# facebookresearch/generative-recommenders

Hardware: AMD Instinct MI355X
Metric: user-seqs/sec (fwd+bwd) HSTU attention L=200 d=512 (higher is better)
Workload: dtype bf16

## Files before the change

### generative_recommenders_amd/csrc/hstu_attn_bwd_fold.cuh

```cuda
#pragma once
#include "hstu_attn_bwd.cuh"

#ifndef FOLD_SDP_AHEAD
#define FOLD_SDP_AHEAD 3
#endif
#ifndef FOLD_DQ32_AHEAD
#define FOLD_DQ32_AHEAD 2
#endif

namespace hstu {

#pragma clang diagnostic push
#pragma clang diagnostic ignored "-Winline-asm"
HSTU_DEV void dma16_asm(const char* g, uint32_t lds_base) {
  asm volatile("s_mov_b32 m0, %1\n\ts_nop 0\n\tglobal_load_lds_dwordx4 %0, off" HSTU_DMA_POLICY ::"v"(g), "s"(lds_base) : "memory", "m0");
}
#pragma clang diagnostic pop

HSTU_DEV void dma16_saddr(uint32_t off, const char* base, uint32_t lds_base) { dma16_saddr_asm(off, base, lds_base); }

template <typename T, int D>
HSTU_DEV void fold_tile_dma(char* tile, const char* base, int64_t row_stride_bytes, int row0, int len, int wave, int lane, bool fast) {
  constexpr int UPR = D * Elem<T>::kBytes / 16;
  constexpr int NCH = 32 * UPR / 64;
  const uint32_t lds0 = __builtin_amdgcn_readfirstlane((uint32_t)(uintptr_t)tile);
  for (int c = wave; c < NCH; c += kBwdWaves) {
    const int pidx = c * 64 + lane;
    const int row = pidx / UPR, slot = pidx % UPR;
    const int unit = slot ^ swz<UPR>(row);
    const int grow = min(row0 + row, len - 1);
    if (fast) dma16_saddr(__umul24((uint32_t)grow, (uint32_t)row_stride_bytes) + unit * 16, base, lds0 + c * 1024);
    else dma16_asm(base + (int64_t)grow * row_stride_bytes + unit * 16, lds0 + c * 1024);
  }
}

HSTU_DEV int fold_ds_off(int row, int chunk) { return (row << 6) + ((chunk ^ ((row >> 1) & 7)) << 3); }

struct FoldNoBias {
  static constexpr bool on = false;
};
struct FoldBias {
  static constexpr bool on = true;
  BiasCtx bc;
  float* hpos;
  float* hts;
  char* bcache;
  bool cached;
  TsRun ts_run;
};

template <typename T, int DQK, int DV, typename BX = FoldNoBias, bool PUBLISH = true, bool CTXM = false>
HSTU_DEV void fold_pair_x(const HstuAttnParams& p, const MaskCtx& mc, const char* __restrict__ Kw, const char* __restrict__ Vw,
                        const char* __restrict__ Qs, const char* __restrict__ dOs, char* __restrict__ myds, int i0, int k0, f32x16 (&dk_acc)[DQK / 32],
                        f32x16 (&dv_acc)[DV / 32], int lane, int dmvm, BX& bx HSTU_TRACE_ARG) {
  using C = BwdCfg<T, DQK, DV>;
  using E = Elem<T>;
  using Frag = typename E::Frag;
  const int n32 = lane & 31, hf = lane >> 5;
  const int len = mc.len;
  const int key = k0 + n32;
  const bool key_ok = key < len;
  f32x16 s, dp;
  Frag pb[2], dsb[2];
  int mode;
  const bool plain = mc.simple || (mc.has_targets && mc.win == 0 && mc.ctx == 0 && i0 + 32 <= min(len, mc.max_id));
  if (plain) mode = (k0 < i0 && i0 + 32 <= len) ? 0 : 1;
  else mode = (i0 + 32 <= len && mc.pair_fully_valid(i0, 32, k0, 32)) ? 0 : 2;
  const int key_id = mc.id_of(key);
  const int key_bits = key_ok ? -1 : 0;
  auto mask_init = [&]() {
    int km = -1;
    if (mode == 1) km = ((k0 == i0) ? dmvm : -1) & ((i0 + 32 > len) ? (dmvm >> 16) : -1);
    if (mode == 2) {
      km = 0;
      bool ctx_done = false;
      if constexpr (CTXM) {
        if (mc.ctx > 0) {
#pragma unroll
          for (int r = 0; r < 16; ++r) {
            const int qi = i0 + (r & 3) + 8 * (r >> 2) + 4 * hf;
            km |= (((qi < len) & key_ok & mc.valid_ids(qi, key, mc.id_of(qi), key_id)) ? 1 : 0) << r;
          }
          ctx_done = true;
        }
      }
      if (!ctx_done) {
#pragma unroll
        for (int r = 0; r < 16; ++r) {
          const int qi = i0 + (r & 3) + 8 * (r >> 2) + 4 * hf;
          km |= (mc.keep_bits_noctx(qi, key, key_id) & key_bits & 1) << r;
        }
      }
    }
    const unsigned nk = ~(unsigned)km;
    const unsigned neg = __builtin_bit_cast(unsigned, p.alpha < 0.f ? 1e30f : -1e30f);
#pragma unroll
    for (int r = 0; r < 16; ++r) {
      const int m = ((int)(nk << (31 - r))) >> 31;
      s[r] = __builtin_bit_cast(float, (unsigned)m & neg);
    }
  };
#pragma unroll
  for (int r = 0; r < 16; ++r) dp[r] = 0.f;
  static_assert(DQK == DV, "interleaved S / dP stream");
  {
    constexpr int NM = 2 * C::KGQ, AHEAD = FOLD_SDP_AHEAD;
    Frag fa[AHEAD + 1], fb[AHEAD + 1];
    auto load_item = [&](int m, Frag& a, Frag& bb) {
      const int e0 = hf * (DQK / 2) + (m >> 1) * 8;
      a = lds_row_frag<T, C::UPR_K>((m & 1) ? dOs : Qs, n32, e0);
      bb = lds_row_frag<T, C::UPR_K>((m & 1) ? Vw : Kw, n32, e0);
    };
#pragma unroll
    for (int m = 0; m < AHEAD; ++m) load_item(m, fa[m % (AHEAD + 1)], fb[m % (AHEAD + 1)]);
    __builtin_amdgcn_sched_barrier(0);
#pragma unroll
    for (int m = 0; m < NM; ++m) {
      if (m + AHEAD < NM) load_item(m + AHEAD, fa[(m + AHEAD) % (AHEAD + 1)], fb[(m + AHEAD) % (AHEAD + 1)]);
      if (m & 1) dp = E::mma(fa[m % (AHEAD + 1)], fb[m % (AHEAD + 1)], dp);
      else if (m == 0) {
        if (mode == 0) {
          f32x16 z;
#pragma unroll
          for (int r = 0; r < 16; ++r) z[r] = 0.f;
          s = E::mma(fa[0], fb[0], z);
        } else {
          mask_init();
          s = E::mma(fa[0], fb[0], s);
        }
      } else s = E::mma(fa[m % (AHEAD + 1)], fb[m % (AHEAD + 1)], s);
      __builtin_amdgcn_sched_barrier(0);
    }
  }
  HSTU_MARK(11);
  int t_k32 = 0;
  if constexpr (BX::on) {
    if (bx.bc.small) t_k32 = bx.bc.t32_at(key);
  }
  float ds_keep[BX::on ? 16 : 1];
  int bkt_keep[BX::on ? 16 : 1];
  int pbase_keep[2] = {0, 0};
  auto elem = [&](const int h8) {
    float pv[8], dsv[8];
    float xb[8];
    int bkt[8];
    int pbase = 0;
    if constexpr (BX::on) {
      const BiasCtx& bc = bx.bc;
      const int qt = i0 >> 5, kt = k0 >> 5;
      char* const bslot = bx.bcache + ((((qt * (qt + 1)) >> 1) + kt) * 2 + h8) * 512 + 8 * lane;
      if (bx.cached) {
        const u32x2 w = *LDS_PTR(const u32x2, bslot);
#pragma unroll
        for (int j = 0; j < 8; ++j) bkt[j] = (int)((w[j >> 2] >> (8 * (j & 3))) & 255u);
      } else {
        if (bc.small) {
#pragma unroll
          for (int g = 0; g < 2; ++g) {
            const auto t4 = bc.t32x4_next(i0 + 8 * (2 * h8 + g) + 4 * hf);
#pragma unroll
            for (int j = 0; j < 4; ++j) bkt[4 * g + j] = bc.bucket32(t4[j], t_k32);
          }
        } else {
#pragma unroll
          for (int j = 0; j < 8; ++j) {
            const int r = 8 * h8 + j;
            bkt[j] = bc.bucket(bc.ts_at(i0 + (r & 3) + 8 * (r >> 2) + 4 * hf + 1), bc.ts_at(key));
          }
        }
        u32x2 w = {0u, 0u};
#pragma unroll
        for (int j = 0; j < 8; ++j) w[j >> 2] |= (unsigned)bkt[j] << (8 * (j & 3));
        *LDS_PTR(u32x2, bslot) = w;
      }
      pbase = bc.pos_index(i0 + 16 * h8 + 4 * hf, key);
#pragma unroll
      for (int j = 0; j < 8; ++j) xb[j] = bc.value(pbase - (j & 3) - 8 * (j >> 2), bkt[j]);
    }
    {
      const f32x2 a2 = {p.alpha, p.alpha};
      const f32x2 c2 = {-1.44269504088896340736f * p.alpha, -1.44269504088896340736f * p.alpha};
      const f32x2 nl2 = {-1.44269504088896340736f, -1.44269504088896340736f};
      const f32x2 one2 = {1.f, 1.f};
#pragma unroll
      for (int j = 0; j < 8; j += 2) {
        const int r = 8 * h8 + j;
        const f32x2 sv = {s[r], s[r + 1]}, dpv = {dp[r], dp[r + 1]};
        f32x2 x = sv * a2, t = sv * c2;
        if constexpr (BX::on) {
          const f32x2 bv = {xb[j], xb[j + 1]};
          x = x + bv;
          t = x * nl2;
        }
        const f32x2 e = {__builtin_amdgcn_exp2f(t[0]), __builtin_amdgcn_exp2f(t[1])};
        const f32x2 dn = e + one2;
        const f32x2 sg = {__builtin_amdgcn_rcpf(dn[0]), __builtin_amdgcn_rcpf(dn[1])};
        const f32x2 pr = x * sg;
        const f32x2 dsr = dpv * (pr * (one2 - sg) + sg);
        pv[j] = pr[0]; pv[j + 1] = pr[1];
        dsv[j] = dsr[0]; dsv[j + 1] = dsr[1];
      }
    }
    if constexpr (BX::on) {
      pbase_keep[h8] = pbase;
#pragma unroll
      for (int j = 0; j < 8; ++j) { ds_keep[8 * h8 + j] = dsv[j]; bkt_keep[8 * h8 + j] = bkt[j]; }
    }
    pb[h8] = E::pack8(pv);
    dsb[h8] = E::pack8(dsv);
  };
  elem(0);
  elem(1);
  HSTU_MARK(12);
  {
    constexpr int NM = 2 * 2 * C::DBQ, AHEAD = FOLD_SDP_AHEAD;
    Frag fa[AHEAD + 1];
    auto load_item = [&](int m, Frag& a) {
      const int ks = (m >> 1) & 1, d = m >> 2;
      a = lds_col_frag<T, C::UPR_K>((m & 1) ? Qs : dOs, 16 * ks + 4 * hf, 16 * ks + 8 + 4 * hf, 32 * d, lane);
    };
#pragma unroll
    for (int m = 0; m < AHEAD; ++m) load_item(m, fa[m % (AHEAD + 1)]);
    __builtin_amdgcn_sched_barrier(0);
#pragma unroll
    for (int m = 0; m < NM; ++m) {
      if (m + AHEAD < NM) load_item(m + AHEAD, fa[(m + AHEAD) % (AHEAD + 1)]);
      const int ks = (m >> 1) & 1, d = m >> 2;
      if (m & 1) dk_acc[d] = E::mma(fa[m % (AHEAD + 1)], dsb[ks], dk_acc[d]);
      else dv_acc[d] = E::mma(fa[m % (AHEAD + 1)], pb[ks], dv_acc[d]);
      __builtin_amdgcn_sched_barrier(0);
    }
  }
#pragma unroll
  for (int rq = 0; PUBLISH && rq < 4; ++rq) {
    const u32x4 w = __builtin_bit_cast(u32x4, dsb[rq >> 1].v);
    u32x2 v2 = {w[2 * (rq & 1)], w[2 * (rq & 1) + 1]};
    *LDS_PTR(u32x2, myds + fold_ds_off(n32, hf + 2 * rq)) = v2;
  }
  if constexpr (BX::on) {
#pragma unroll
    for (int h8 = 0; h8 < 2; ++h8) {
      const float* dsv_ = ds_keep + 8 * h8;
      const int* bkt_ = bkt_keep + 8 * h8;
      const int pbase_ = pbase_keep[h8];
      const int p16 = lane & 15;
#pragma unroll
      for (int gg = 0; gg < 2; ++gg) {
        float t = dsv_[4 * gg + 3];
#pragma unroll
        for (int j = 2; j >= 0; --j)
          t = __builtin_bit_cast(float, __builtin_amdgcn_update_dpp(0, __builtin_bit_cast(int, t), 0x101, 0xf, 0xf, true)) + dsv_[4 * gg + j];
        if (t != 0.f) atomicAdd(bx.hpos + pbase_ - 8 * gg, t);
#pragma unroll
        for (int j = 1; j < 4; ++j)
          if (p16 < j && dsv_[4 * gg + j] != 0.f) atomicAdd(bx.hpos + pbase_ - 8 * gg - j, dsv_[4 * gg + j]);
      }
      if (bx.bc.lts) {
#pragma unroll
        for (int j = 0; j < 8; ++j) bx.ts_run.add(bkt_[j], dsv_[j]);
      }
    }
  }
}

template <typename T, int DQK, int DV>
HSTU_DEV void fold_pair(const HstuAttnParams& p, const MaskCtx& mc, const char* __restrict__ Kw, const char* __restrict__ Vw,
                        const char* __restrict__ Qs, const char* __restrict__ dOs, char* __restrict__ myds, int i0, int k0, f32x16 (&dk_acc)[DQK / 32],
                        f32x16 (&dv_acc)[DV / 32], int lane, int dmvm HSTU_TRACE_ARG) {
  FoldNoBias nb;
  fold_pair_x<T, DQK, DV, FoldNoBias>(p, mc, Kw, Vw, Qs, dOs, myds, i0, k0, dk_acc, dv_acc, lane, dmvm, nb HSTU_TRACE_PASS);
}

template <typename T, int D>
HSTU_DEV void fold_park_tile(const f32x16 (&acc)[D / 32], float scale, char* __restrict__ tile, int lane) {
  constexpr int UPR = D * Elem<T>::kBytes / 16;
  const int n32 = lane & 31, hf = lane >> 5;
#pragma unroll
  for (int d = 0; d < D / 32; ++d)
#pragma unroll
    for (int rq = 0; rq < 4; ++rq) {
      u32x2 v = {Elem<T>::pk2(acc[d][4 * rq] * scale, acc[d][4 * rq + 1] * scale),
                 Elem<T>::pk2(acc[d][4 * rq + 2] * scale, acc[d][4 * rq + 3] * scale)};
      *LDS_PTR(u32x2, tile + tile_off<UPR>(n32, 4 * d + rq) + 8 * hf) = v;
    }
}
template <typename T, int D, int NT = kBwdThreads>
HSTU_DEV void fold_copy_out(const char* __restrict__ tile, char* gtile, int64_t row_stride_bytes, int rows_valid, int tid) {
  constexpr int UPR = D * Elem<T>::kBytes / 16;
  for (int u = tid; u < 32 * UPR; u += NT) {
    const int row = u / UPR, unit = u % UPR;
    const u32x4 v = *LDS_PTR(const u32x4, tile + tile_off<UPR>(row, unit));
    if (row < rows_valid) gstore16_nt(gtile + row * row_stride_bytes + unit * 16, v);
  }
}

template <int NB>
HSTU_DEV void fold_dump(const f32x16 (&acc)[NB], char* __restrict__ region, int lane) {
#pragma unroll
  for (int d = 0; d < NB; ++d)
#pragma unroll
    for (int c = 0; c < 4; ++c) {
      f32x4 v4 = {acc[d][4 * c], acc[d][4 * c + 1], acc[d][4 * c + 2], acc[d][4 * c + 3]};
      *LDS_PTR(f32x4, region + ((d * 4 + c) * 64 + lane) * 16) = v4;
    }
}
template <int NB>
HSTU_DEV void fold_add(f32x16 (&acc)[NB], const char* __restrict__ region, int lane) {
#pragma unroll
  for (int d = 0; d < NB; ++d)
#pragma unroll
    for (int c = 0; c < 4; ++c) {
      const f32x4 v4 = *LDS_PTR(const f32x4, region + ((d * 4 + c) * 64 + lane) * 16);
#pragma unroll
      for (int e = 0; e < 4; ++e) acc[d][4 * c + e] += v4[e];
    }
}

template <typename T>
HSTU_DEV typename Elem<T>::Frag tr_frag16(const char* base, int off_lo, int off_hi) {
  s16x4 a = __builtin_amdgcn_ds_read_tr16_b64_v4i16(LDS_PTR(s16x4, base + off_lo));
  s16x4 b = __builtin_amdgcn_ds_read_tr16_b64_v4i16(LDS_PTR(s16x4, base + off_hi));
  typedef short s16x8 __attribute__((ext_vector_type(8)));
  s16x8 ab = {a[0], a[1], a[2], a[3], b[0], b[1], b[2], b[3]};
  typename Elem<T>::Frag f;
  f.v = __builtin_bit_cast(typename Elem<T>::vec8, ab);
  return f;
}

template <typename T, int DQK, int DV, int NA, int NB>
HSTU_DEV void fold_dq_slots(char* dq_head, int64_t dq_rs, const MaskCtx& mc, const char* __restrict__ kv,
                            const char* __restrict__ dsbuf, int a, int bq, bool b_on, int wave,
                            float ds_scale, int lane HSTU_TRACE_ARG) {
  using C = BwdCfg<T, DQK, DV>;
  using F = FoldCfg<T, DQK, DV>;
  using E = Elem<T>;
  using Frag = typename E::Frag;
  const int db = wave & 3, qb = wave >> 2;
  if (db >= DQK / 32) return;
  const int i16 = lane & 15, g = lane >> 4;
  const int row_lo = 8 * g + (i16 >> 2), row_hi = row_lo + 4;
  constexpr bool kContig = C::UPR_K == 16;
  const int colK0 = kContig ? 32 * db + 4 * (i16 & 3) : 32 * db + 8 * (i16 & 3), colK1 = colK0 + (kContig ? 16 : 4);
  const int k0_lo = tile_off<C::UPR_K>(row_lo, colK0 >> 3) + ((colK0 & 7) << 1);
  const int k0_hi = tile_off<C::UPR_K>(row_hi, colK0 >> 3) + ((colK0 & 7) << 1);
  const int k1_lo = tile_off<C::UPR_K>(row_lo, colK1 >> 3) + ((colK1 & 7) << 1);
  const int k1_hi = tile_off<C::UPR_K>(row_hi, colK1 >> 3) + ((colK1 & 7) << 1);
  const int d_lo = fold_ds_off(row_lo, 4 * qb + (i16 & 3)), d_hi = fold_ds_off(row_hi, 4 * qb + (i16 & 3));
  unsigned on_a = (1u << (a + 1)) - 1u, on_b = b_on ? (1u << (bq + 1)) - 1u : 0u;
  if (mc.win != 0) {
    for (int t = 0; t <= a; ++t)
      if (!mc.pair_may_be_active(32 * a, 32, 32 * t, 32)) on_a &= ~(1u << t);
    if (b_on)
      for (int t = 0; t <= bq; ++t)
        if (!mc.pair_may_be_active(32 * bq, 32, 32 * t, 32)) on_b &= ~(1u << t);
  }
  HSTU_MARK(19);
  f32x4 acc[2][2];
#pragma unroll
  for (int sd = 0; sd < 2; ++sd)
#pragma unroll
    for (int h = 0; h < 2; ++h) acc[sd][h] = f32x4{0.f, 0.f, 0.f, 0.f};
  const u32x4 zero4 = {0u, 0u, 0u, 0u};
#pragma unroll
  for (int sd = 0; sd < 2; ++sd) {
#pragma unroll
    for (int t = 0; t < (sd ? NB : NA); ++t) {
      const bool on = ((sd ? on_b : on_a) >> t) & 1u;
      const char* Kt = kv + t * C::PAIR;
      const char* ds = dsbuf + (sd ? (kBwdWaves - 1 - t) : t) * F::DSB;
      const Frag fk0 = tr_frag16<T>(Kt, k0_lo, k0_hi), fk1 = tr_frag16<T>(Kt, k1_lo, k1_hi);
      Frag fd = tr_frag16<T>(ds, d_lo, d_hi);
      fd.v = __builtin_bit_cast(typename E::vec8, on ? __builtin_bit_cast(u32x4, fd.v) : zero4);
      acc[sd][0] = E::mma16(fk0, fd, acc[sd][0]);
      acc[sd][1] = E::mma16(fk1, fd, acc[sd][1]);
    }
  }
  {
    constexpr int NSLOT = NA + NB;
    __builtin_amdgcn_sched_group_barrier(0x100, 6, 0);
#pragma unroll
    for (int sl = 0; sl < NSLOT; ++sl) {
      if (sl + 1 < NSLOT) __builtin_amdgcn_sched_group_barrier(0x100, 6, 0);
      __builtin_amdgcn_sched_group_barrier(0x002, 4, 0);
      __builtin_amdgcn_sched_group_barrier(0x008, 2, 0);
    }
  }
  HSTU_MARK(16);
#pragma unroll
  for (int sd = 0; sd < 2; ++sd) {
    if (sd == 1 && !b_on) break;
    uint32_t x0 = E::pk2(acc[sd][0][0] * ds_scale, acc[sd][0][1] * ds_scale), x1 = E::pk2(acc[sd][0][2] * ds_scale, acc[sd][0][3] * ds_scale);
    uint32_t y0 = E::pk2(acc[sd][1][0] * ds_scale, acc[sd][1][1] * ds_scale), y1 = E::pk2(acc[sd][1][2] * ds_scale, acc[sd][1][3] * ds_scale);
    int f0 = 8 * g;
    if constexpr (kContig) {
      const auto s0 = __builtin_amdgcn_permlane16_swap(x0, y0, false, false);
      const auto s1 = __builtin_amdgcn_permlane16_swap(x1, y1, false, false);
      x0 = s0[0]; y0 = s0[1]; x1 = s1[0]; y1 = s1[1];
      f0 = 8 * (2 * (g & 1) + (g >> 1));
    }
    const int qrow = 32 * (sd ? bq : a) + 16 * qb + i16;
    if (qrow < mc.len) gstore16(dq_head + qrow * dq_rs + (32 * db + f0) * C::EB, u32x4{x0, x1, y0, y1});
  }
}

template <typename T, int DQK, int DV>
HSTU_DEV void fold_dq_phase(char* dq_head, int64_t dq_rs, const MaskCtx& mc, const char* __restrict__ kv,
                            const char* __restrict__ dsbuf, int a, int bq, bool b_on, int wave,
                            float ds_scale, int lane HSTU_TRACE_ARG) {
#define HSTU_FOLD_DQ(NA_, NB_) return fold_dq_slots<T, DQK, DV, NA_, NB_>(dq_head, dq_rs, mc, kv, dsbuf, a, bq, b_on, wave, ds_scale, lane HSTU_TRACE_PASS)
  const int code = 8 * (a + 1) + (b_on ? bq + 1 : 0);
  switch (code) {
    case 8 * 7 + 1: HSTU_FOLD_DQ(7, 1);
    case 8 * 6 + 2: HSTU_FOLD_DQ(6, 2);
    case 8 * 5 + 3: HSTU_FOLD_DQ(5, 3);
    case 8 * 4 + 0: HSTU_FOLD_DQ(4, 0);
    default: HSTU_FOLD_DQ(7, 4);
  }
#undef HSTU_FOLD_DQ
}

template <typename T, int D, int N>
HSTU_DEV f32x16 fold_dq_chain32(const char* __restrict__ kv, const char* __restrict__ ds0, int ds_step, int db, int lane) {
  using C = BwdCfg<T, D, D>;
  using E = Elem<T>;
  using Frag = typename E::Frag;
  const int hf = lane >> 5, i16 = lane & 15, g1 = (lane >> 4) & 1;
  const int ra = 8 * hf, rb = 16 + 8 * hf;
  const int chunk = 4 * g1 + (i16 & 3), rr = i16 >> 2;
  const int o00 = fold_ds_off(ra + rr, chunk), o01 = fold_ds_off(ra + 4 + rr, chunk);
  const int o10 = fold_ds_off(rb + rr, chunk), o11 = fold_ds_off(rb + 4 + rr, chunk);
  f32x16 acc;
#pragma unroll
  for (int r = 0; r < 16; ++r) acc[r] = 0.f;
#pragma unroll
  for (int t = 0; t < N; ++t) {
    const char* Kt = kv + t * C::PAIR;
    const char* ds = ds0 + t * ds_step;
    const Frag a0 = lds_col_frag<T, C::UPR_K>(Kt, ra, ra + 4, 32 * db, lane);
    const Frag a1 = lds_col_frag<T, C::UPR_K>(Kt, rb, rb + 4, 32 * db, lane);
    const Frag b0 = tr_frag16<T>(ds, o00, o01);
    const Frag b1 = tr_frag16<T>(ds, o10, o11);
    acc = E::mma(a0, b0, acc);
    acc = E::mma(a1, b1, acc);
  }
  {
    constexpr int AH = FOLD_DQ32_AHEAD < N ? FOLD_DQ32_AHEAD : N;
    __builtin_amdgcn_sched_group_barrier(0x100, 8 * AH, 0);
#pragma unroll
    for (int t = 0; t < N; ++t) {
      if (t + AH < N) __builtin_amdgcn_sched_group_barrier(0x100, 8, 0);
      __builtin_amdgcn_sched_group_barrier(0x008, 2, 0);
    }
  }
  return acc;
}

template <typename T, int D>
HSTU_DEV void fold_dq_phase32(char* dq_head, int64_t dq_rs, const MaskCtx& mc, const char* __restrict__ kv, const char* __restrict__ dsbuf,
                              int a, int bq, bool b_on, int wave, float ds_scale, int lane HSTU_TRACE_ARG) {
  using C = BwdCfg<T, D, D>;
  using F = FoldCfg<T, D, D>;
  using E = Elem<T>;
  static_assert(D == 128, "four feature blocks x two sides = eight waves");
  const int db = wave & 3, side = wave >> 2;
  if (side == 1 && !b_on) return;
  const int n = side ? bq + 1 : a + 1;
  const int q0 = 32 * (side ? bq : a);
  const char* ds0 = side ? dsbuf + (kBwdWaves - 1) * F::DSB : dsbuf;
  const int ds_step = side ? -F::DSB : F::DSB;
  HSTU_MARK(19);
  f32x16 acc;
  switch (n) {
    case 1: acc = fold_dq_chain32<T, D, 1>(kv, ds0, ds_step, db, lane); break;
    case 2: acc = fold_dq_chain32<T, D, 2>(kv, ds0, ds_step, db, lane); break;
    case 3: acc = fold_dq_chain32<T, D, 3>(kv, ds0, ds_step, db, lane); break;
    case 4: acc = fold_dq_chain32<T, D, 4>(kv, ds0, ds_step, db, lane); break;
    case 5: acc = fold_dq_chain32<T, D, 5>(kv, ds0, ds_step, db, lane); break;
    case 6: acc = fold_dq_chain32<T, D, 6>(kv, ds0, ds_step, db, lane); break;
    default: acc = fold_dq_chain32<T, D, 7>(kv, ds0, ds_step, db, lane); break;
  }
  HSTU_MARK(16);
  const int n32 = lane & 31, hf = lane >> 5;
  uint32_t g[4][2];
#pragma unroll
  for (int j = 0; j < 4; ++j) {
    g[j][0] = E::pk2(acc[4 * j] * ds_scale, acc[4 * j + 1] * ds_scale);
    g[j][1] = E::pk2(acc[4 * j + 2] * ds_scale, acc[4 * j + 3] * ds_scale);
  }
#pragma unroll
  for (int jp = 0; jp < 4; jp += 2)
#pragma unroll
    for (int h = 0; h < 2; ++h) {
      const auto sw = __builtin_amdgcn_permlane32_swap(g[jp][h], g[jp + 1][h], false, false);
      g[jp][h] = sw[0];
      g[jp + 1][h] = sw[1];
    }
  const int qrow = q0 + n32;
  if (qrow < mc.len) {
    char* dst = dq_head + qrow * dq_rs + (32 * db + 8 * hf) * C::EB;
    gstore16(dst, u32x4{g[0][0], g[0][1], g[1][0], g[1][1]});
    gstore16(dst + 16 * C::EB, u32x4{g[2][0], g[2][1], g[3][0], g[3][1]});
  }
}


typedef const __attribute__((address_space(4))) uint32_t* kargw_t;
#define HSTU_KARG(k, field) (((const __attribute__((address_space(4))) HstuAttnBwdParams*)(k))->field)

HSTU_DEV HstuAttnBwdParams reload_bwd_params(kargw_t k) {
  static_assert(sizeof(HstuAttnBwdParams) % 4 == 0, "word copy");
  HstuAttnBwdParams r;
  uint32_t* d = (uint32_t*)&r;
#pragma unroll
  for (int i = 0; i < (int)(sizeof(HstuAttnBwdParams) / 4); ++i) d[i] = k[i];
  return r;
}

struct FoldWork {
  int64_t off0;
  int len;
  int b, hd;
};

HSTU_DEV FoldWork fold_work(const HstuAttnParams& p, int uh, int tmax) {
  FoldWork w;
  w.b = user_of_slot_s(p, uh / p.heads);
  w.hd = uh % p.heads;
  w.off0 = sload_index(p.seq_offsets, w.b, p.offsets_dtype);
  w.len = min((int)(sload_index(p.seq_offsets, w.b + 1, p.offsets_dtype) - w.off0), 32 * tmax);
  return w;
}

template <typename T, int DQK, int DV, typename BX = FoldNoBias>
HSTU_DEV void fold_problem_x(const HstuAttnBwdParams& bp, kargw_t kargs, int tmax, const FoldWork& cur, const FoldWork& nxt, char* smem,
                             int tid, int lane, int wave, int& pre_lo, BX& bx) {
  using C = BwdCfg<T, DQK, DV>;
  using F = FoldCfg<T, DQK, DV>;
  static_assert(C::EB == 2, "the folded backward is built for 16-bit I/O");
  static_assert(DQK / 32 <= 4, "dQ GEMM: 32 feature columns x 16 query rows per wave");
  static_assert(DQK == DV, "hand-over regions assume equal K and V tile sizes");
  const HstuAttnParams& p = bp.fwd;
  const int64_t off0 = cur.off0;
  const int len = cur.len, hd = cur.hd;
  const int pre_in = pre_lo;
  pre_lo = F::kMaxTiles;
  if (len <= 0) return;
  const MaskCtx mc = make_mask_ctx<true>(p, cur.b, len);
  HSTU_TRACE_DECL(bp.workspace, bp.workspace != nullptr && cur.b * p.heads + hd == 4096);
  HSTU_MARK(1);

  const int nt = (len + 31) >> 5;
  const int ns = (nt + 1) >> 1;
  char* const stageA = smem + F::kMaxTiles * C::PAIR;
  char* const stageB = stageA + C::PAIR;
  char* const dsbuf = stageB + C::PAIR;

  const char* qbase = (const char*)p.q + (off0 * p.q_row_stride + (int64_t)hd * p.q_head_stride) * C::EB;
  const char* dobase = (const char*)bp.dout + (off0 * bp.do_row_stride + (int64_t)hd * bp.do_head_stride) * C::EB;
  char* const dq_head = (char*)bp.dq + (off0 * bp.dq_row_stride + (int64_t)hd * bp.dq_head_stride) * C::EB;
  char* const dk_head = (char*)bp.dk + (off0 * bp.dk_row_stride + (int64_t)hd * bp.dk_head_stride) * C::EB;
  char* const dv_head = (char*)bp.dv + (off0 * bp.dv_row_stride + (int64_t)hd * bp.dv_head_stride) * C::EB;
  const int64_t dq_rs = bp.dq_row_stride * C::EB, dk_rs = bp.dk_row_stride * C::EB, dv_rs = bp.dv_row_stride * C::EB;
  const int64_t q_rs = p.q_row_stride * C::EB, k_rs = p.k_row_stride * C::EB, v_rs = p.v_row_stride * C::EB,
                do_rs = bp.do_row_stride * C::EB;

  const int len_max = 32 * tmax;
  const bool dma_fast = q_rs < (1 << 24) && k_rs < (1 << 24) && v_rs < (1 << 24) && do_rs < (1 << 24) &&
                        (int64_t)len_max * q_rs < (1LL << 32) && (int64_t)len_max * k_rs < (1LL << 32) &&
                        (int64_t)len_max * v_rs < (1LL << 32) && (int64_t)len_max * do_rs < (1LL << 32);
  auto stage_dma = [&](int qa, int qb, bool b_on) {
    fold_tile_dma<T, DQK>(stageA, qbase, q_rs, 32 * qa, len, wave, lane, dma_fast);
    fold_tile_dma<T, DV>(stageA + C::KT, dobase, do_rs, 32 * qa, len, wave, lane, dma_fast);
    if (b_on) {
      fold_tile_dma<T, DQK>(stageB, qbase, q_rs, 32 * qb, len, wave, lane, dma_fast);
      fold_tile_dma<T, DV>(stageB + C::KT, dobase, do_rs, 32 * qb, len, wave, lane, dma_fast);
    }
  };

  {
    const char* kbase = (const char*)p.k + (off0 * p.k_row_stride + (int64_t)hd * p.k_head_stride) * C::EB;
    const char* vbase = (const char*)p.v + (off0 * p.v_row_stride + (int64_t)hd * p.v_head_stride) * C::EB;
    for (int t = 0; t < min(nt, pre_in); ++t) {
      char* dst = smem + t * C::PAIR;
      fold_tile_dma<T, DQK>(dst, kbase, k_rs, 32 * t, len, wave, lane, dma_fast);
      fold_tile_dma<T, DV>(dst + C::KT, vbase, v_rs, 32 * t, len, wave, lane, dma_fast);
    }
  }
  stage_dma(nt - 1, 0, 0 < nt - 1);
  for (int i = tid; i < kBwdWaves * F::DSB / 16; i += kBwdThreads) *LDS_PTR(u32x4, dsbuf + 16 * i) = u32x4{0u, 0u, 0u, 0u};
  for (int t = nt; t < F::kMaxTiles; ++t)
    for (int i = tid; i < C::KT / 16; i += kBwdThreads) *LDS_PTR(u32x4, smem + t * C::PAIR + 16 * i) = u32x4{0u, 0u, 0u, 0u};
  HSTU_MARK(2);

  f32x16 dk_acc[C::DBQ], dv_acc[C::DBV];
#pragma unroll
  for (int d = 0; d < C::DBQ; ++d)
#pragma unroll
    for (int r = 0; r < 16; ++r) dk_acc[d][r] = 0.f;
#pragma unroll
  for (int d = 0; d < C::DBV; ++d)
#pragma unroll
    for (int r = 0; r < 16; ++r) dv_acc[d][r] = 0.f;
  const float scale_v = attn_scale_of(p);
  const float ds_scale = scale_v * p.alpha;

  int dmvm = 0;
  {
    const int n32 = lane & 31, hf = lane >> 5;
#pragma unroll
    for (int r = 0; r < 16; ++r) {
      const int row = (r & 3) + 8 * (r >> 2) + 4 * hf;
      dmvm |= (n32 <= row ? 1 : 0) << r;
      dmvm |= (32 * (nt - 1) + row < len ? 1 : 0) << (16 + r);
    }
  }

  for (int k = 0; k < ns; ++k) {
    const int a = nt - 1 - k, bq = k;
    const bool b_on = bq < a;
    asm volatile("s_waitcnt vmcnt(0)" ::: "memory");
    __syncthreads();
    HSTU_MARK(10);
    if (k > 0 && wave == a + 1) {
      int lane3 = lane;
      asm volatile("" : "+v"(lane3));
      fold_park_tile<T, DQK>(dk_acc, ds_scale, smem + wave * C::PAIR, lane3);
#pragma unroll
      for (int d = 0; d < C::DBQ; ++d)
#pragma unroll
        for (int r = 0; r < 16; ++r) dk_acc[d][r] = 0.f;
    }
    int kt = -1, qt = 0;
    const char* st = stageA;
    if (wave <= a) { kt = wave; qt = a; }
    else if (b_on && kBwdWaves - 1 - wave <= bq) { kt = kBwdWaves - 1 - wave; qt = bq; st = stageB; }
    if (kt >= 0 && (mc.win == 0 || mc.pair_may_be_active(32 * qt, 32, 32 * kt, 32))) {
      const char* Kw = smem + kt * C::PAIR;
      int lane1 = lane;
      asm volatile("" : "+v"(lane1));
      fold_pair_x<T, DQK, DV, BX>(p, mc, Kw, Kw + C::KT, st, st + C::KT, dsbuf + wave * F::DSB, 32 * qt, 32 * kt, dk_acc,
                                  dv_acc, lane1, dmvm, bx HSTU_TRACE_PASS);
    }
    HSTU_MARK(13);
    HSTU_MARK(14);
    __syncthreads();
    HSTU_MARK(15);
    if (k + 1 < ns) stage_dma(a - 1, bq + 1, bq + 1 < a - 1);
    if (k > 0) {
      const int kt1 = a + 1;
      fold_copy_out<T, DQK>(smem + kt1 * C::PAIR, dk_head + (int64_t)(32 * kt1) * dk_rs, dk_rs, len - 32 * kt1, tid);
      fold_copy_out<T, DV>(smem + kt1 * C::PAIR + C::KT, dv_head + (int64_t)(32 * kt1) * dv_rs, dv_rs, len - 32 * kt1, tid);
    }
    HSTU_MARK(18);
    int lane2 = lane;
    asm volatile("" : "+v"(lane2));
    bool done32 = false;
    if constexpr (DQK == 128 && DV == 128 && !BX::on) {
      if (mc.win == 0) {
        fold_dq_phase32<T, DQK>(dq_head, dq_rs, mc, smem, dsbuf, a, bq, b_on, wave, ds_scale, lane2 HSTU_TRACE_PASS);
        done32 = true;
      }
    }
    if (!done32) fold_dq_phase<T, DQK, DV>(dq_head, dq_rs, mc, smem, dsbuf, a, bq, b_on, wave, ds_scale, lane2 HSTU_TRACE_PASS);
    HSTU_MARK(17);
    if (kt == wave && wave == a) {
      int lane3 = lane;
      asm volatile("" : "+v"(lane3));
      fold_park_tile<T, DV>(dv_acc, scale_v, smem + wave * C::PAIR + C::KT, lane3);
#pragma unroll
      for (int d = 0; d < C::DBV; ++d)
#pragma unroll
        for (int r = 0; r < 16; ++r) dv_acc[d][r] = 0.f;
    }
    HSTU_MARK(23);
  }
  HSTU_MARK(20);
  const int nb = nt >> 1;
  const int a_last = nt - ns;
  const int bt = kBwdWaves - 1 - wave;
  const bool a_fin = wave < nb, b_fin = bt < nb;
  const int tb = a_fin ? wave : bt;
  char* const reg_a = smem + tb * C::PAIR;
  char* const reg_b = tb == 0 ? stageA : (tb == 1 ? stageB : dsbuf);
  __syncthreads();
  if (nxt.len > 0) {
    kargw_t k2 = kargs;
    asm volatile("" : "+s"(k2));
    const int64_t krs3 = HSTU_KARG(k2, fwd.k_row_stride), vrs3 = HSTU_KARG(k2, fwd.v_row_stride);
    const char* kb3 = (const char*)HSTU_KARG(k2, fwd.k) + (nxt.off0 * krs3 + (int64_t)nxt.hd * HSTU_KARG(k2, fwd.k_head_stride)) * C::EB;
    const char* vb3 = (const char*)HSTU_KARG(k2, fwd.v) + (nxt.off0 * vrs3 + (int64_t)nxt.hd * HSTU_KARG(k2, fwd.v_head_stride)) * C::EB;
    const int nt3 = (nxt.len + 31) >> 5;
    for (int t = a_last + 1; t < nt3; ++t) {
      char* dst = smem + t * C::PAIR;
      fold_tile_dma<T, DQK>(dst, kb3, krs3 * C::EB, 32 * t, nxt.len, wave, lane, dma_fast);
      fold_tile_dma<T, DV>(dst + C::KT, vb3, vrs3 * C::EB, 32 * t, nxt.len, wave, lane, dma_fast);
    }
    pre_lo = a_last + 1;
  }
  int lane4 = lane;
  asm volatile("" : "+v"(lane4));
  if (wave == a_last) fold_park_tile<T, DQK>(dk_acc, ds_scale, smem + wave * C::PAIR, lane4);
  if (a_fin) fold_dump<C::DBV>(dv_acc, reg_a, lane4);
  if (b_fin) fold_dump<C::DBQ>(dk_acc, reg_b, lane4);
  __syncthreads();
  HSTU_MARK(22);
  if (a_fin) {
    fold_add<C::DBQ>(dk_acc, reg_b, lane4);
    fold_park_tile<T, DQK>(dk_acc, ds_scale, reg_b, lane4);
  }
  if (b_fin) {
    fold_add<C::DBV>(dv_acc, reg_a, lane4);
    fold_park_tile<T, DV>(dv_acc, scale_v, reg_a + C::KT, lane4);
  }
  __syncthreads();
  HSTU_MARK(24);
  fold_copy_out<T, DQK>(smem + a_last * C::PAIR, dk_head + (int64_t)(32 * a_last) * dk_rs, dk_rs, len - 32 * a_last, tid);
  fold_copy_out<T, DV>(smem + a_last * C::PAIR + C::KT, dv_head + (int64_t)(32 * a_last) * dv_rs, dv_rs, len - 32 * a_last, tid);
  for (int t = 0; t < nb; ++t) {
    const char* rb = t == 0 ? stageA : (t == 1 ? stageB : dsbuf);
    fold_copy_out<T, DQK>(rb, dk_head + (int64_t)(32 * t) * dk_rs, dk_rs, len - 32 * t, tid);
    fold_copy_out<T, DV>(smem + t * C::PAIR + C::KT, dv_head + (int64_t)(32 * t) * dv_rs, dv_rs, len - 32 * t, tid);
  }
  HSTU_MARK(21);
}

template <typename T, int DQK, int DV>
__global__ __launch_bounds__(kBwdThreads) __attribute__((amdgpu_waves_per_eu(2, 2))) void hstu_attn_bwd_fold_kernel(const HstuAttnBwdParams bp_arg, int tmax) {
  extern __shared__ __attribute__((aligned(16))) char smem[];
  const int tid = threadIdx.x;
  const int lane = tid & 63;
  const int wave = __builtin_amdgcn_readfirstlane(tid >> 6);
  const kargw_t kargs = (kargw_t)__builtin_amdgcn_kernarg_segment_ptr();
  const int total = HSTU_KARG(kargs, fwd.batch) * HSTU_KARG(kargs, fwd.heads);
  int pre_lo = 7;
  FoldNoBias nb;
  FoldWork cur;
  {
    const HstuAttnBwdParams bp0 = reload_bwd_params(kargs);
    cur = fold_work(bp0.fwd, blockIdx.x, tmax);
  }
  for (int uh = blockIdx.x; uh < total; uh += gridDim.x) {
    kargw_t kl = kargs;
    asm volatile("" : "+s"(kl));
    const HstuAttnBwdParams bp = reload_bwd_params(kl);
    FoldWork nxt;
    nxt.len = 0; nxt.off0 = 0; nxt.b = 0; nxt.hd = 0;
    if (uh + (int)gridDim.x < total) nxt = fold_work(bp.fwd, uh + (int)gridDim.x, tmax);
    fold_problem_x<T, DQK, DV, FoldNoBias>(bp, kl, tmax, cur, nxt, smem, tid, lane, wave, pre_lo, nb);
    cur = nxt;
    __syncthreads();
  }
}

template <typename T, int D>
__global__ __launch_bounds__(kBwdThreads) __attribute__((amdgpu_waves_per_eu(2, 2))) void hstu_attn_bwd_fold_bias_kernel(
    const HstuAttnBwdParams bp_arg, int tmax, float* bias_partial, int ts_copies, int hist_bytes, int table_bytes, int* next_user) {
  using F = FoldCfg<T, D, D>;
  extern __shared__ __attribute__((aligned(16))) char smem[];
  const int tid = threadIdx.x;
  const int lane = tid & 63;
  const int wave = __builtin_amdgcn_readfirstlane(tid >> 6);
  const kargw_t kargs = (kargw_t)__builtin_amdgcn_kernarg_segment_ptr();
  const int batch = HSTU_KARG(kargs, fwd.batch), heads = HSTU_KARG(kargs, fwd.heads);
  const int max_seq_len = HSTU_KARG(kargs, fwd.max_seq_len), num_buckets = HSTU_KARG(kargs, fwd.num_buckets);
  FoldBias bx;
  bx.hpos = (float*)(smem + F::smem_bytes());
  bx.hts = bx.hpos + 2 * max_seq_len;
  char* const tables = (char*)bx.hpos + hist_bytes;
  bx.bcache = tables + table_bytes;
  bx.ts_run.init(bx.hts, ts_copies);
  bx.cached = false;
  const int hist_floats = 2 * max_seq_len + (num_buckets + 1) * ts_copies;
  for (int i = tid; i < hist_floats; i += kBwdThreads) bx.hpos[i] = 0.f;
  int pre_lo = 7;
  FoldWork cur;
  {
    const HstuAttnBwdParams bp0 = reload_bwd_params(kargs);
    cur = fold_work(bp0.fwd, (int)blockIdx.x * heads, tmax);
  }
  volatile int* const slot = (volatile int*)(bx.hpos + 2 * max_seq_len - 1);
  int ticket = 0;
  if (tid == 0) ticket = (int)gridDim.x + atomicAdd(next_user, 1);
  for (int u = blockIdx.x; u < batch;) {
    if (tid == 0) {
      *slot = ticket;
      ticket = (int)gridDim.x + atomicAdd(next_user, 1);
    }
    __syncthreads();
    {
      kargw_t kl = kargs;
      asm volatile("" : "+s"(kl));
      const HstuAttnBwdParams bp = reload_bwd_params(kl);
      bx.bc = stage_bias_tables(bp.fwd, cur.b, tables, tid, kBwdThreads, u != (int)blockIdx.x);
    }
    __syncthreads();
    bx.bc.finish(kBwdWaves);
    const int u_next = __builtin_amdgcn_readfirstlane(*slot);
    for (int hd = 0; hd < heads; ++hd) {
      kargw_t kl = kargs;
      asm volatile("" : "+s"(kl));
      const HstuAttnBwdParams bp = reload_bwd_params(kl);
      const int uh = u * heads + hd;
      const int uh_n = hd + 1 < heads ? uh + 1 : (u_next < batch ? u_next * heads : -1);
      FoldWork nxt;
      nxt.len = 0; nxt.off0 = 0; nxt.b = 0; nxt.hd = 0;
      if (hd + 1 < heads) { nxt = cur; nxt.hd = hd + 1; }
      else if (uh_n >= 0) nxt = fold_work(bp.fwd, uh_n, tmax);
      bx.cached = hd > 0;
      fold_problem_x<T, D, D, FoldBias>(bp, kl, tmax, cur, nxt, smem, tid, lane, wave, pre_lo, bx);
      cur = nxt;
      __syncthreads();
    }
    u = u_next;
  }
  bx.ts_run.flush();
  __syncthreads();
  const HstuAttnBwdParams bp = reload_bwd_params(kargs);
  const float scale_v = attn_scale_of(bp.fwd);
  float* row = bias_partial + (int64_t)blockIdx.x * (2 * max_seq_len + num_buckets);
  const int npos = 2 * max_seq_len - 1;
  for (int i = tid; i < 2 * max_seq_len + num_buckets; i += kBwdThreads) {
    float v;
    if (i < npos) {
      v = bx.hpos[i];
    } else {
      v = 0.f;
      const float* cp = bx.hts + (i - npos) * ts_copies;
      for (int c = 0; c < ts_copies; ++c) v += cp[c];
    }
    row[i] = v * scale_v;
  }
}

}
```

Measured before the change: 1.922 million.

## Add software-pipelined pair kernel interleaving S/dP, dV and dK MFMA streams

Adds an alternate fold_pair_x path, selected at compile time, that runs the S/dP MMAs and the following dV/dK MMAs as one unrolled stream with fragment loads issued ahead. The sigmoid/P and dS elementwise stages are placed among the MMAs according to a configurable ordering, and dS publication to LDS is delayed. The aim is to hide LDS load latency and elementwise SFU work behind matrix-core work. It is enabled by default with order 3 for DQK=128 without bias, and it raises register pressure from the larger prefetch and staging arrays.

```diff
diff --git a/generative_recommenders_amd/csrc/hstu_attn_bwd_fold.cuh b/generative_recommenders_amd/csrc/hstu_attn_bwd_fold.cuh
--- a/generative_recommenders_amd/csrc/hstu_attn_bwd_fold.cuh
+++ b/generative_recommenders_amd/csrc/hstu_attn_bwd_fold.cuh
@@ -49,7 +49,39 @@
   TsRun ts_run;
 };
 
-template <typename T, int DQK, int DV, typename BX = FoldNoBias, bool PUBLISH = true, bool CTXM = false>
+#ifndef FOLD_PAIR_ORDER
+#define FOLD_PAIR_ORDER 3
+#endif
+#ifndef FOLD_PAIR_PACKED
+#define FOLD_PAIR_PACKED 0
+#endif
+#ifndef FOLD_PAIR_LEAD
+#define FOLD_PAIR_LEAD 3
+#endif
+template <int ORDER, int KGQ, int DB>
+struct FoldPairOrder {
+  static constexpr int NS = 2 * KGQ, ND = 4 * DB, N = NS + ND;
+  static constexpr int L = FOLD_PAIR_LEAD;
+  static constexpr int SLAST = ORDER == 4 ? 2 * KGQ - 2 - L : (ORDER == 1 ? KGQ - 1 : 2 * KGQ - 2);
+  static constexpr int kind(int pos) {
+    if (pos < NS) {
+      if (ORDER == 1) return pos >= KGQ ? 1 : 0;
+      if (ORDER == 4) return pos < L ? 0 : (pos > SLAST ? 1 : ((pos - L) & 1));
+      return pos & 1;
+    }
+    const int m = pos - NS;
+    return 2 + (ORDER == 1 ? (m >= 2 * DB ? 1 : 0) : (m & 1));
+  }
+  static constexpr int kq(int pos) {
+    if (ORDER == 1) return pos % KGQ;
+    if (ORDER == 4) return pos < L ? pos : (pos > SLAST ? KGQ - 1 - L + (pos - SLAST - 1) : (((pos - L) & 1) ? (pos - L - 1) / 2 : L + (pos - L) / 2));
+    return pos >> 1;
+  }
+  static constexpr int d(int pos) { return ORDER == 1 ? (pos - NS) % DB : ((pos - NS) >> 1) % DB; }
+  static constexpr int ks(int pos) { return ORDER == 1 ? ((pos - NS) / DB) & 1 : (pos - NS) / (2 * DB); }
+};
+
+template <typename T, int DQK, int DV, typename BX = FoldNoBias, bool PUBLISH = true, bool CTXM = false, int ORDER = 0>
 HSTU_DEV void fold_pair_x(const HstuAttnParams& p, const MaskCtx& mc, const char* __restrict__ Kw, const char* __restrict__ Vw,
                         const char* __restrict__ Qs, const char* __restrict__ dOs, char* __restrict__ myds, int i0, int k0, f32x16 (&dk_acc)[DQK / 32],
                         f32x16 (&dv_acc)[DV / 32], int lane, int dmvm, BX& bx HSTU_TRACE_ARG) {
@@ -103,6 +135,139 @@
 #pragma unroll
   for (int r = 0; r < 16; ++r) dp[r] = 0.f;
   static_assert(DQK == DV, "interleaved S / dP stream");
+  if constexpr (ORDER != 0) {
+    static_assert(!BX::on && E::kBytes == 2, "pipelined pair: 16-bit I/O, no bias");
+    using PO = FoldPairOrder<ORDER, C::KGQ, C::DBQ>;
+    constexpr int AHEAD = FOLD_SDP_AHEAD, NS = PO::NS, N = PO::N, NG = 2 * C::DBQ;
+    static_assert(16 % C::KGQ == 0 && 16 % NG == 0 && (16 / C::KGQ) % 2 == 0 && (16 / NG) % 2 == 0, "element pairs per slot");
+    Frag fa[AHEAD + 1], fb[AHEAD + 1];
+    float fac[16];
+    uint32_t pw[8], dsw[8];
+    auto load_item = [&](int pos, Frag& a, Frag& bb) {
+      const int kd = PO::kind(pos);
+      if (kd < 2) {
+        const int e0 = hf * (DQK / 2) + PO::kq(pos) * 8;
+        a = lds_row_frag<T, C::UPR_K>(kd ? dOs : Qs, n32, e0);
+        bb = lds_row_frag<T, C::UPR_K>(kd ? Vw : Kw, n32, e0);
+      } else {
+        const int ks = PO::ks(pos), d = PO::d(pos);
+        a = lds_col_frag<T, C::UPR_K>(kd == 3 ? Qs : dOs, 16 * ks + 4 * hf, 16 * ks + 8 + 4 * hf, 32 * d, lane);
+      }
+    };
+    auto frag_of = [&](const uint32_t* w) {
+      Frag f;
+      f.v = __builtin_bit_cast(typename E::vec8, u32x4{w[0], w[1], w[2], w[3]});
+      return f;
+    };
+    auto stage1 = [&](int r) {
+#if FOLD_PAIR_PACKED
+      const f32x2 a2 = {p.alpha, p.alpha};
+      const f32x2 c2 = {-1.44269504088896340736f * p.alpha, -1.44269504088896340736f * p.alpha};
+      const f32x2 one2 = {1.f, 1.f};
+      const f32x2 sv = {s[r], s[r + 1]};
+      const f32x2 x = sv * a2, t = sv * c2;
+      const f32x2 e = {__builtin_amdgcn_exp2f(t[0]), __builtin_amdgcn_exp2f(t[1])};
+      const f32x2 dn = e + one2;
+      const f32x2 sg = {__builtin_amdgcn_rcpf(dn[0]), __builtin_amdgcn_rcpf(dn[1])};
+      const f32x2 pr = x * sg;
+      const f32x2 f2 = pr * (one2 - sg) + sg;
+      fac[r] = f2[0]; fac[r + 1] = f2[1];
+      pw[r >> 1] = E::pk2(pr[0], pr[1]);
+#else
+      float pr[2];
+#pragma unroll
+      for (int j = 0; j < 2; ++j) {
+        const float x = s[r + j] * p.alpha, t = s[r + j] * (-1.44269504088896340736f * p.alpha);
+        const float sg = __builtin_amdgcn_rcpf(__builtin_amdgcn_exp2f(t) + 1.f);
+        pr[j] = x * sg;
+        fac[r + j] = pr[j] * (1.f - sg) + sg;
+      }
+      pw[r >> 1] = E::pk2(pr[0], pr[1]);
+#endif
+    };
+    auto stage2 = [&](int r) {
+#if FOLD_PAIR_PACKED
+      const f32x2 dpv = {dp[r], dp[r + 1]}, f2 = {fac[r], fac[r + 1]};
+      const f32x2 dsr = dpv * f2;
+      dsw[r >> 1] = E::pk2(dsr[0], dsr[1]);
+#else
+      dsw[r >> 1] = E::pk2(dp[r] * fac[r], dp[r + 1] * fac[r + 1]);
+#endif
+    };
+    auto publish = [&](int rq) {
+      if constexpr (PUBLISH) {
+        u32x2 v2 = {dsw[2 * rq], dsw[2 * rq + 1]};
+        *LDS_PTR(u32x2, myds + fold_ds_off(n32, hf + 2 * rq)) = v2;
+      }
+    };
+#pragma unroll
+    for (int m = 0; m < AHEAD; ++m) load_item(m, fa[m % (AHEAD + 1)], fb[m % (AHEAD + 1)]);
+    __builtin_amdgcn_sched_barrier(0);
+#pragma unroll
+    for (int pos = 0; pos < N; ++pos) {
+      if (pos + AHEAD < N) load_item(pos + AHEAD, fa[(pos + AHEAD) % (AHEAD + 1)], fb[(pos + AHEAD) % (AHEAD + 1)]);
+      const Frag &a = fa[pos % (AHEAD + 1)], &bb = fb[pos % (AHEAD + 1)];
+      const int kd = PO::kind(pos);
+      if (kd == 1) dp = E::mma(a, bb, dp);
+      else if (kd == 0) {
+        if (PO::kq(pos) == 0) {
+          if (mode == 0) {
+            f32x16 z;
+#pragma unroll
+            for (int r = 0; r < 16; ++r) z[r] = 0.f;
+            s = E::mma(a, bb, z);
+          } else {
+            mask_init();
+            s = E::mma(a, bb, s);
+          }
+        } else s = E::mma(a, bb, s);
+      } else if (kd == 2) dv_acc[PO::d(pos)] = E::mma(a, frag_of(pw + 4 * PO::ks(pos)), dv_acc[PO::d(pos)]);
+      else dk_acc[PO::d(pos)] = E::mma(a, frag_of(dsw + 4 * PO::ks(pos)), dk_acc[PO::d(pos)]);
+      if constexpr (ORDER == 1) {
+        constexpr int E1 = 16 / C::KGQ, E2 = 16 / NG;
+        const int g1 = pos - C::KGQ - 1, g2 = pos - NS - 1;
+        if (g1 >= 0 && g1 < C::KGQ)
+#pragma unroll
+          for (int r = g1 * E1; r < (g1 + 1) * E1; r += 2) stage1(r);
+        if (g2 >= 0 && g2 < NG)
+#pragma unroll
+          for (int r = g2 * E2; r < (g2 + 1) * E2; r += 2) stage2(r);
+      } else {
+        const int g = pos - NS;
+        constexpr int PER = NG / 4;
+        static_assert(PER >= 1, "four element pairs under the ks = 0 items");
+        if (ORDER != 3 && g >= 0 && g < NG) {
+          if (g % PER == 0) stage1(8 + 2 * (g / PER));
+          if (g % PER == PER - 1) stage2(8 + 2 * (g / PER));
+        }
+        if constexpr (ORDER == 4) {
+          constexpr int TS = NS - 1 - PO::SLAST;
+          const int t = pos - PO::SLAST - 1;
+          if (t >= 0 && t < TS)
+#pragma unroll
+            for (int q = 0; q < 4; ++q)
+              if ((q * TS) / 4 == t) stage1(2 * q);
+        }
+      }
+#pragma unroll
+      for (int rq = 0; rq < 4; ++rq)
+        if ((NS + NG + 1 + rq < N - 1 ? NS + NG + 1 + rq : N - 1) == pos) publish(rq);
+      __builtin_amdgcn_sched_barrier(0);
+      if (pos == NS - 1) {
+        HSTU_MARK(11);
+        if constexpr (ORDER != 1) {
+#pragma unroll
+          for (int r = 0; r < (ORDER == 3 ? 16 : 8); r += 2) {
+            if (ORDER != 4) stage1(r);
+            stage2(r);
+          }
+          __builtin_amdgcn_sched_barrier(0);
+        }
+      }
+      if (pos == (ORDER == 1 ? NS + NG : NS + NG - 1)) HSTU_MARK(12);
+    }
+    return;
+  }
   {
     constexpr int NM = 2 * C::KGQ, AHEAD = FOLD_SDP_AHEAD;
     Frag fa[AHEAD + 1], fb[AHEAD + 1];
@@ -638,8 +803,9 @@
       const char* Kw = smem + kt * C::PAIR;
       int lane1 = lane;
       asm volatile("" : "+v"(lane1));
-      fold_pair_x<T, DQK, DV, BX>(p, mc, Kw, Kw + C::KT, st, st + C::KT, dsbuf + wave * F::DSB, 32 * qt, 32 * kt, dk_acc,
-                                  dv_acc, lane1, dmvm, bx HSTU_TRACE_PASS);
+      constexpr int kOrder = (DQK == 128 && !BX::on) ? FOLD_PAIR_ORDER : 0;
+      fold_pair_x<T, DQK, DV, BX, true, false, kOrder>(p, mc, Kw, Kw + C::KT, st, st + C::KT, dsbuf + wave * F::DSB, 32 * qt, 32 * kt, dk_acc,
+                                                       dv_acc, lane1, dmvm, bx HSTU_TRACE_PASS);
     }
     HSTU_MARK(13);
     HSTU_MARK(14);
```

Result: slower. 1.899 million (-1.2%).
